# samkatt/fba-pomdp

Measured on AMD Instinct MI355X. Metric: simulated env steps/sec (belief+rollout), higher is better.
Workload: dtype f64

## Files before the change

fba_pomdp_amd/csrc/fba_search.hip:

```cpp
#include <algorithm>
#include <cstdio>
#include <cstdlib>
#include <cstring>

#include "fba_kernels_common.h"

namespace fba {

__device__ __forceinline__ int et_reward_code(double r) { return r == -1.0 ? 0 : (r == 10.0 ? 1 : 2); }
__device__ __forceinline__ double et_reward(int code) { return code == 0 ? -1.0 : (code == 1 ? 10.0 : -100.0); }
#ifdef FBA_PROFILE_SEARCH
__device__ unsigned long long g_search_prof[12];
#define PROF_MARK(r) { const long long now_ = clock64(); prof_[r] += now_ - prev_; prev_ = now_; }
#else
#define PROF_MARK(r)
#endif
template <bool STAGE, int AMAX, bool REG, int TIGER_TABLE, int MODEL, int FTIGER = 0, bool TIGER_POMDP = false, bool FTP = false, bool ETIGER = false>
__global__ void __launch_bounds__(SEARCH_BLOCK) search_kernel(Problem P, DeviceState D)
{
    if (TIGER_POMDP) {
        P.S = 2; P.A = 3; P.O = 2; P.C = 0; P.Cs = 4; P.planner = FBA_PLANNER_POUCT;
        if (P.domain != FBA_DOM_TIGER_CONTINUOUS) P.domain = FBA_DOM_TIGER_EPISODIC;
        P.belief = P.belief == FBA_BELIEF_IMPORTANCE ? FBA_BELIEF_IMPORTANCE : FBA_BELIEF_REJECTION;
        D.cn_off = 1; D.cq_off = 4; D.child_off = 10; D.node_words = 16; D.hash = nullptr;
    }
    P.model = MODEL;
    if (FTIGER > 0) {
        P.S = 1 << FTIGER; P.A = 3; P.O = 2;
        if (P.domain != FBA_DOM_FTIGER_CONTINUOUS) P.domain = FBA_DOM_FTIGER_EPISODIC;
        if (ETIGER) P.domain = FBA_DOM_FTIGER_EPISODIC;
    }
    if (ETIGER) { P.A = 3; P.O = 2; }
    if (TIGER_TABLE) {
        P.model = FBA_MODEL_BA_TABLE; P.planner = FBA_PLANNER_POUCT;
        P.S = 2; P.A = 3; P.O = 2; P.phi_len = 12; P.C = 24; P.Cs = 32;
        if (P.domain != FBA_DOM_TIGER_CONTINUOUS) P.domain = FBA_DOM_TIGER_EPISODIC;
        P.belief = P.belief == FBA_BELIEF_IMPORTANCE ? FBA_BELIEF_IMPORTANCE : FBA_BELIEF_REJECTION;
        D.cn_off = 1; D.cq_off = 4; D.child_off = 10; D.node_words = 16; D.hash = nullptr;
        if (TIGER_TABLE == 2) { P.C = 12; P.Cs = 16; }
    }
    if (ETIGER && (TIGER_TABLE || TIGER_POMDP)) P.domain = FBA_DOM_TIGER_EPISODIC;
    extern __shared__ double lds[];
    __shared__ __attribute__((aligned(8))) float s_prior[TIGER_TABLE == 2 ? 24 : 2];
    const int lane = threadIdx.x;
    const int e    = blockIdx.x * SEARCH_BLOCK + lane;
    if (TIGER_TABLE == 2) {
        if (lane < 24) s_prior[lane] = D.prior_dense[lane];
        __syncthreads();
    }
    if (MODEL == FBA_MODEL_BA_FACTORED && FTIGER == 0) {
        size_t words = search_lds_words(P, D, STAGE, ETIGER);
        words = (words + 3) & ~(size_t)3;
        uint4* dst       = reinterpret_cast<uint4*>(reinterpret_cast<uint32_t*>(lds) + words);
        const uint4* src = reinterpret_cast<const uint4*>(P.fd);
        for (int k = lane; k < (P.fd_bytes + 15) / 16; k += SEARCH_BLOCK) dst[k] = src[k];
        __syncthreads();
        P.fd = reinterpret_cast<const FDesc*>(dst);
    }
    if (e >= P.E || !D.active[e]) return;

    const int depth_cap = P.max_depth > 0 ? P.max_depth : 1;
    float* path_r       = reinterpret_cast<float*>(lds) + lane;
    int32_t* path_na    = reinterpret_cast<int32_t*>(path_r - lane + (size_t)depth_cap * SEARCH_BLOCK) + lane;
    uint16_t* path16    = reinterpret_cast<uint16_t*>(lds) + lane;
    float* stage        = ETIGER ? reinterpret_cast<float*>(lds) + (size_t)((depth_cap + 1) / 2) * SEARCH_BLOCK + lane
                                 : reinterpret_cast<float*>(path_na - lane + (size_t)depth_cap * SEARCH_BLOCK) + lane;
    const bool root_lds = !ETIGER && root_children_in_lds(P, D);
    int16_t* rootch     = reinterpret_cast<int16_t*>(stage - lane + (STAGE ? (size_t)P.Cs * SEARCH_BLOCK : 0)) + lane;
    uint32_t* l1        = reinterpret_cast<uint32_t*>(stage - lane + (STAGE ? (size_t)P.Cs * SEARCH_BLOCK : 0)) + lane;

    Rng g               = slot_rng(P, D, e);
    const int hist_len  = D.t[e];
    const int max_tree_depth = min(P.horizon - hist_len, P.max_depth);
    const int W         = D.node_words;
    int32_t* tree       = D.nodes + (size_t)e * D.max_nodes * W;
    const float* prec   = D.p_rec + pbase(P, e, D.bufsel[e]) * (size_t)P.Cs;

    const bool nested = TIGER_TABLE != 2 && !TIGER_POMDP && !FTP && MODEL != FBA_MODEL_POMDP && P.nested != 0;
    if (P.planner == FBA_PLANNER_RANDOM) {
        g.stream(FBA_PHASE_SEARCH, (uint32_t)P.sims);
        int ns = 0;
        const int src = nested ? nested_sample(P, D, e, g, ns) : belief_sample_uniform(P, D, g);
        D.action[e]   = domain_random_action(P, g, nested ? ns : slot_lazy(D, e) ? lazy_state(P, D, e, src) : rec_state(prec + (size_t)src * P.Cs, P.C));
        return;
    }

    node_init(D, tree, P.A, P.O);
    int n_nodes = 1, tree_depth = 0;
    unsigned long long steps = 0;
    int r_vis = 0, r_cn[AMAX];
    double r_cq[AMAX];
#pragma unroll
    for (int a = 0; a < AMAX; ++a) { r_cn[a] = 0; r_cq[a] = 0.0; }
    if (root_lds)
        for (int k = 0; k < P.A * P.O; ++k) rootch[k * SEARCH_BLOCK] = -1;
    uint32_t l1_exists = 0;
    int4 cy_h2 = make_int4(0, 0, 0, 0), cy_h3 = make_int4(0, 0, 0, 0);
    double cy_q2 = 0, cy_q3 = 0;
    int4* tab      = hash_table(D, e);
    const uint32_t epoch = D.hash ? hash_begin_search(D, e, tab, 0, 1) : 0;

    constexpr bool COMPACT = TIGER_TABLE == 2 && ETIGER;
    const int lazy_c = (slot_lazy(D, e) ? 1 : 0) | (COMPACT && D.compact[e] ? 2 : 0);
    if (COMPACT && (lazy_c & 2)) {
#pragma unroll
        for (int w = 0; w < 10; ++w)
            if (w != 2 && w != 5) stage[w * SEARCH_BLOCK] = 0.f;
    }
    int ts_src = -1, ts_state = 0;
    if (P.planner == FBA_PLANNER_TS) {
        g.stream(FBA_PHASE_SEARCH, (uint32_t)P.sims + 2u);
        ts_src = nested ? nested_sample(P, D, e, g, ts_state) : belief_sample_uniform(P, D, g);
    }
    int sim = -1, mode = 0;
    int s = 0, node = 0, dtg = 0, plen = 0, rdepth = 0;
    const float* cnt = prec;
    double rret = 0, rdisc = 1;
    const int quorum = D.search_quorum;
#ifdef FBA_PROFILE_SEARCH
    long long prof_[12] = {0, 0, 0, 0, 0, 0, 0, 0, 0, 0, 0, 0}, prev_ = clock64();
#endif
    while (true) {
        PROF_MARK(6)
        const bool waiting = mode == 0 && sim < P.sims;
        const int n_wait = __popcll(__ballot(waiting)), n_act = __popcll(__ballot(mode != 0));
        if (n_wait + n_act == 0) break;
        const bool boundary = n_act == 0 || n_wait * 64 >= quorum * (n_wait + n_act);
#ifdef FBA_PROFILE_SEARCH
        const bool lead_ = lane == __ffsll((unsigned long long)__ballot(true)) - 1;
        if (lead_) { prof_[5] += 1; if (boundary) { prof_[9] += 1; prof_[10] += n_wait; } }
#endif
        if (boundary && waiting) {
            double del = rret;
            for (int k = plen - 1; k >= (ETIGER ? 4 : 1); --k) {
                const int na     = ETIGER ? (int)path16[(size_t)k * SEARCH_BLOCK] : path_na[(size_t)k * SEARCH_BLOCK];
                const double ret = (ETIGER ? et_reward(na >> 14) : (double)path_r[(size_t)k * SEARCH_BLOCK]) + P.gamma * del;
                const int act    = ETIGER ? ((na >> 12) & 3) : (na & 31);
                int32_t* rec = tree + (size_t)(ETIGER ? (na & 0xfff) : (na >> 5)) * W;
                double* q    = reinterpret_cast<double*>(rec + D.cq_off) + act;
                int n;
                if (P.A == 3) {
                    int4* hp = reinterpret_cast<int4*>(rec);
                    int4 h   = *hp;
                    n = act == 0 ? ++h.y : (act == 1 ? ++h.z : ++h.w);
                    ++h.x;
                    *hp = h;
                } else {
                    n = ++rec[D.cn_off + act];
                    if (D.cn_off) ++rec[0];
                }
                *q += (ret - *q) / (double)n;
                del = ret;
            }
            if (ETIGER) {
#pragma unroll
                for (int lv = 3; lv >= 2; --lv)
                    if (plen > lv) {
                        const int na     = (int)path16[(size_t)lv * SEARCH_BLOCK];
                        const double ret = et_reward(na >> 14) + P.gamma * del;
                        const int act    = (na >> 12) & 3;
                        int32_t* rec     = tree + (size_t)(na & 0xfff) * W;
                        int4 h           = lv == 3 ? cy_h3 : cy_h2;
                        const double q0  = lv == 3 ? cy_q3 : cy_q2;
                        const int n      = act == 0 ? ++h.y : (act == 1 ? ++h.z : ++h.w);
                        ++h.x;
                        *reinterpret_cast<int4*>(rec) = h;
                        reinterpret_cast<double*>(rec + D.cq_off)[act] = q0 + (ret - q0) / (double)n;
                        del = ret;
                    }
            }
            if (ETIGER && plen > 1) {
                const int na     = (int)path16[1 * SEARCH_BLOCK];
                const double ret = et_reward(na >> 14) + P.gamma * del;
                const int act    = (na >> 12) & 3;
                uint32_t* nd     = l1 + (size_t)(na & 0xfff) * ET_NODE_WORDS * SEARCH_BLOCK;
                uint32_t* cw     = nd + (act >> 1) * SEARCH_BLOCK;
                const uint32_t w = *cw;
                const int n      = (int)((act & 1) ? (w >> 16) : (w & 0xffffu)) + 1;
                *cw              = (act & 1) ? ((w & 0xffffu) | ((uint32_t)n << 16)) : ((w & 0xffff0000u) | (uint32_t)n);
                uint32_t* qw     = nd + (size_t)(3 + 2 * act) * SEARCH_BLOCK;
                double q         = __hiloint2double((int)qw[SEARCH_BLOCK], (int)qw[0]);
                q += (ret - q) / (double)n;
                qw[0]            = (uint32_t)__double2loint(q);
                qw[SEARCH_BLOCK] = (uint32_t)__double2hiint(q);
                del = ret;
            }
            if (plen > 0) {
                const double ret = (ETIGER ? et_reward((int)path16[0] >> 14) : (double)path_r[0]) + P.gamma * del;
                const int act    = ETIGER ? (((int)path16[0] >> 12) & 3) : (path_na[0] & 31);
                int n = 0;
                double q = 0.0;
#pragma unroll
                for (int a2 = 0; a2 < AMAX; ++a2)
                    if (a2 == act) { n = r_cn[a2]; q = r_cq[a2]; }
                ++n;
                q += (ret - q) / (double)n;
#pragma unroll
                for (int a2 = 0; a2 < AMAX; ++a2)
                    if (a2 == act) { r_cn[a2] = n; r_cq[a2] = q; }
                ++r_vis;
            }
            ++sim;
            plen = 0;
        }
        PROF_MARK(4)
        if (boundary && waiting && sim < P.sims) {
            g.stream(FBA_PHASE_SEARCH, (uint32_t)sim);
            int nest_state = ts_state;
            const int src = ts_src >= 0 ? ts_src : (nested ? nested_sample(P, D, e, g, nest_state) : belief_sample_uniform(P, D, g));
            cnt = prec + (size_t)src * P.Cs;
            if (COMPACT && (lazy_c & 2)) {
                const uint4 v = reinterpret_cast<const uint4*>(prec)[src];
                stage[2 * SEARCH_BLOCK]  = __uint_as_float(v.x);
                stage[5 * SEARCH_BLOCK]  = __uint_as_float(v.y);
                stage[10 * SEARCH_BLOCK] = __uint_as_float(v.z);
                stage[11 * SEARCH_BLOCK] = __uint_as_float(v.w & 0x7fffffffu);
                s = (int)(v.w >> 31);
                stage[12 * SEARCH_BLOCK] = __int_as_float(s);
            } else if (STAGE) {
                const float4* rp = reinterpret_cast<const float4*>(cnt);
                const int n4 = (P.C + 4) >> 2;
                constexpr int NB = TIGER_TABLE == 2 ? 4 : 12;
                for (int k0 = 0; k0 < n4; k0 += NB) {
                    float4 v[NB];
#pragma unroll
                    for (int q = 0; q < NB; ++q) v[q] = rp[min(k0 + q, n4 - 1)];
#pragma unroll
                    for (int q = 0; q < NB; ++q) {
                        const int k = k0 + q;
                        if (k < n4) {
                            stage[(4 * k + 0) * SEARCH_BLOCK] = v[q].x;
                            stage[(4 * k + 1) * SEARCH_BLOCK] = v[q].y;
                            stage[(4 * k + 2) * SEARCH_BLOCK] = v[q].z;
                            stage[(4 * k + 3) * SEARCH_BLOCK] = v[q].w;
                        }
                    }
                }
                s = __float_as_int(stage[P.C * SEARCH_BLOCK]);
            } else {
                s = rec_state(cnt, P.C);
            }
            if (lazy_c & 1) s = lazy_state(P, g, src);
            if (nested) s = nest_state;
            node = 0; dtg = max_tree_depth; plen = 0; mode = 1;
        }
        PROF_MARK(0)
        bool finish = false, do_step = mode != 0;
        double delayed = 0;
        int a = 0;
        if (mode == 1) {
            tree_depth = max(tree_depth, max_tree_depth - dtg);
            if (dtg == 0) { finish = true; do_step = false; }
            else if (ETIGER) {
                int cn[AMAX], vis = r_vis;
                double cq[AMAX];
#pragma unroll
                for (int a2 = 0; a2 < AMAX; ++a2) { cn[a2] = r_cn[a2]; cq[a2] = r_cq[a2]; }
                if (node < 0) {
                    const uint32_t* nd = l1 + (size_t)(-1 - node) * ET_NODE_WORDS * SEARCH_BLOCK;
                    const uint32_t w0 = nd[0], w1 = nd[1 * SEARCH_BLOCK];
                    cn[0] = (int)(w0 & 0xffffu); cn[1] = (int)(w0 >> 16); cn[2] = (int)(w1 & 0xffffu);
#pragma unroll
                    for (int a2 = 0; a2 < 3; ++a2)
                        cq[a2] = __hiloint2double((int)nd[(4 + 2 * a2) * SEARCH_BLOCK], (int)nd[(3 + 2 * a2) * SEARCH_BLOCK]);
                    vis = (cn[0] + cn[1]) + cn[2];
                } else if (node > 0) {
                    const int32_t* rec = tree + (size_t)node * W;
                    const int4 h      = *reinterpret_cast<const int4*>(rec);
                    const double2 q01 = *reinterpret_cast<const double2*>(rec + 4);
                    const double q2   = *reinterpret_cast<const double*>(rec + 8);
                    vis = h.x; cn[0] = h.y; cn[1] = h.z; cn[2] = h.w;
                    cq[0] = q01.x; cq[1] = q01.y; cq[2] = q2;
                }
                a = ucb_pick<AMAX>(P, g, D.log1p_tab, vis, cn, cq, true);
                if (plen == 2) { cy_h2 = make_int4(vis, cn[0], cn[1], cn[2]); cy_q2 = a == 0 ? cq[0] : (a == 1 ? cq[1] : cq[2]); }
                if (plen == 3) { cy_h3 = make_int4(vis, cn[0], cn[1], cn[2]); cy_q3 = a == 0 ? cq[0] : (a == 1 ? cq[1] : cq[2]); }
            }
            else if (node == 0) a = ucb_pick<AMAX>(P, g, D.log1p_tab, r_vis, r_cn, r_cq, true);
            else a = ucb_select<AMAX>(P, D, g, tree + (size_t)node * W, true);
        } else if (mode == 2) {
            a = domain_random_action(P, g, s);
        }
        PROF_MARK(1)
        int o;
        double r;
        bool term;
        if (do_step) {
            if (FTIGER > 0 && STAGE && FTP)
                term = ftiger_step_packed<(FTIGER > 0 ? FTIGER : 1)>(P, g, LdsView<SEARCH_BLOCK>{stage}, s, a, o, r, NoInc{});
            else if (FTIGER > 0 && STAGE) term = ftiger_step<(FTIGER > 0 ? FTIGER : 1)>(P, g, LdsView<SEARCH_BLOCK>{stage}, s, a, o, r, NoInc{});
            else if (FTIGER > 0) term = ftiger_step<(FTIGER > 0 ? FTIGER : 1)>(P, g, GlobalSearchView{cnt}, s, a, o, r, NoInc{});
            else if (TIGER_TABLE == 2)
                term = tiger_step_packed(P, g, [&](int w) { return __float_as_uint(stage[w * SEARCH_BLOCK]); }, s_prior, s, a, o, r, NoInc{});
            else if (STAGE) term = sim_step<REG>(P, g, LdsView<SEARCH_BLOCK>{stage}, s, a, o, r, NoInc{});
            else term = sim_step<REG>(P, g, GlobalSearchView{cnt}, s, a, o, r, NoInc{});
            ++steps;
#ifdef FBA_PROFILE_SEARCH
        }
        PROF_MARK(2)
        if (do_step) {
#endif
            if (ETIGER && mode == 1) {
                path16[(size_t)plen * SEARCH_BLOCK] = (uint16_t)((node < 0 ? -1 - node : node) | (a << 12) | (et_reward_code(r) << 14));
                ++plen;
                if (term) finish = true;
                else {
                    int c = 0;
                    if (node == 0) c = ((l1_exists >> o) & 1u) ? -1 - o : 0;
                    else if (node < 0) {
                        const uint32_t w2 = l1[((size_t)(-1 - node) * ET_NODE_WORDS + 2) * SEARCH_BLOCK];
                        c = (int)(o ? (w2 >> 16) : (w2 & 0xffffu));
                    } else {
                        c = tree[(size_t)node * W + D.child_off + 2 * 2 + o];
                        c = c < 0 ? 0 : c;
                    }
                    if (c != 0) { node = c; --dtg; }
                    else {
                        const int nn = min(n_nodes, D.max_nodes - 1);
                        ++n_nodes;
                        if (node == 0) {
                            uint32_t* nd = l1 + (size_t)o * ET_NODE_WORDS * SEARCH_BLOCK;
#pragma unroll
                            for (int k = 0; k < ET_NODE_WORDS; ++k) nd[k * SEARCH_BLOCK] = 0;
                            l1_exists |= 1u << o;
                        } else {
                            node_init(D, tree + (size_t)nn * W, P.A, P.O);
                            if (node < 0) {
                                uint32_t* w2 = l1 + ((size_t)(-1 - node) * ET_NODE_WORDS + 2) * SEARCH_BLOCK;
                                *w2 = o ? ((*w2 & 0xffffu) | ((uint32_t)nn << 16)) : ((*w2 & 0xffff0000u) | (uint32_t)nn);
                            } else tree[(size_t)node * W + D.child_off + 2 * 2 + o] = nn;
                        }
                        mode = 2; rdepth = dtg - 1; rret = 0; rdisc = 1;
                        if (rdepth == 0) finish = true;
                    }
                }
            } else if (mode == 1) {
                path_r[(size_t)plen * SEARCH_BLOCK]  = (float)r;
                path_na[(size_t)plen * SEARCH_BLOCK] = (node << 5) | a  ;
                ++plen;
                if (term) finish = true;
                else {
                    const bool at_root_lds = root_lds && node == 0;
                    const int c = at_root_lds ? rootch[(a * P.O + o) * SEARCH_BLOCK] : child_get(P, D, tree, tab, epoch, node, a, o);
                    if (c >= 0) { node = c; --dtg; }
                    else {
                        const int nn = min(n_nodes, D.max_nodes - 1);
                        ++n_nodes;
                        node_init(D, tree + (size_t)nn * W, P.A, P.O);
                        if (at_root_lds) rootch[(a * P.O + o) * SEARCH_BLOCK] = (int16_t)nn;
                        else child_set(P, D, tree, tab, epoch, node, a, o, nn);
                        mode = 2; rdepth = dtg - 1; rret = 0; rdisc = 1;
                        if (rdepth == 0) finish = true;
                    }
                }
            } else {
                rret += r * rdisc;
                rdisc *= P.gamma;
                --rdepth;
                if (rdepth == 0 || term) { delayed = rret; finish = true; }
            }
        }
        PROF_MARK(3)
        if (finish) { rret = delayed; mode = 0; }
#ifdef FBA_PROFILE_SEARCH
        {
            const int n_step_ = __popcll(__ballot(do_step));
            if (lead_) prof_[8] += n_step_;
        }
#endif
    }
#ifdef FBA_PROFILE_SEARCH
    for (int r = 0; r < 12; ++r)
        if ((r == 5 || r >= 8 ? prof_[r] != 0 : lane == 0) && r != 7 && r != 11) atomicAdd(&g_search_prof[r], (unsigned long long)prof_[r]);
#endif
    g.stream(FBA_PHASE_SEARCH, (uint32_t)P.sims + 1u);
    if (n_nodes > D.max_nodes) atomicCAS(D.fault, 0, -(1 + e));
    const int best = ucb_pick<AMAX>(P, g, D.log1p_tab, 0, r_cn, r_cq, false);
    D.action[e]    = best;
    D.sim_steps[e] += steps;
    fba_trace_rec& rec = D.cur[e];
    rec.n_nodes    = n_nodes;
    rec.tree_depth = tree_depth;
#pragma unroll
    for (int a = 0; a < FBA_MAX_ACTIONS; ++a) {
        rec.root_n[a] = a < AMAX && a < P.A ? r_cn[a < AMAX ? a : 0] : 0;
        rec.root_q[a] = a < AMAX && a < P.A ? r_cq[a < AMAX ? a : 0] : 0.0;
    }
}

template <int K>
__global__ void __launch_bounds__(SEARCH_BLOCK) search_hist_kernel(Problem P, DeviceState D)
{
    constexpr int AMAX = 4;
    P.model = FBA_MODEL_BA_FACTORED; P.domain = FBA_DOM_GRIDWORLD; P.A = 4; P.belief = FBA_BELIEF_IMPORTANCE;
    extern __shared__ double lds[];
    const int lane = threadIdx.x, tl = lane >> 2;
    const int e    = blockIdx.x * HIST_TREES + tl;
    if (e >= P.E || !D.active[e]) return;

    const int depth_cap = P.max_depth > 0 ? P.max_depth : 1;
    double* path_q   = lds + tl;
    int32_t* path_n  = reinterpret_cast<int32_t*>(path_q - tl + (size_t)depth_cap * HIST_TREES) + tl;
    float* path_r    = reinterpret_cast<float*>(path_n - tl + (size_t)depth_cap * HIST_TREES) + tl;
    int32_t* path_na = reinterpret_cast<int32_t*>(path_r - tl + (size_t)depth_cap * HIST_TREES) + tl;
    uint32_t* stage  = reinterpret_cast<uint32_t*>(path_na - tl + (size_t)depth_cap * HIST_TREES) + tl;
    const bool carry = D.cn_off == 0;
    const bool spec = carry && D.max_nodes <= 65538 && P.sims <= 65536;
    int pf_node = -1;
    int4 pf_h = make_int4(0, 0, 0, 0);
    double2 pf_q01 = make_double2(0, 0), pf_q23 = make_double2(0, 0);
    int r_hint[AMAX] = {0, 0, 0, 0};

    QuadRng g;
    g.init(P.seed_lo, P.seed_hi, (uint32_t)D.run[e], (uint32_t)D.episode[e], (uint32_t)D.t[e], lane);
    const int hist_len  = D.t[e];
    const int max_tree_depth = min(P.horizon - hist_len, P.max_depth);
    const int W         = D.node_words;
    int32_t* tree       = D.nodes + (size_t)e * D.max_nodes * W;
    const float* prec   = D.p_rec + rec_base(P, D, e, D.bufsel[e]) * (size_t)P.Cs;
    const uint32_t hist_cnt = D.hist_cnt[e];
    const int hist_n        = hist_total(hist_cnt);
    const uint32_t hist_off = (uint32_t)hist_offset(hist_cnt, 1) << 8 | (uint32_t)hist_offset(hist_cnt, 2) << 16 | (uint32_t)hist_offset(hist_cnt, 3) << 24;

    if (P.planner == FBA_PLANNER_RANDOM) {
        g.stream(FBA_PHASE_SEARCH, (uint32_t)P.sims);
        g.ensure(2);
        (void)g.u01();
        D.action[e] = g.slow_int(0, 4);
        if (P.search_budget > 0) D.search_done[e] = 1;
        return;
    }
    const int budget  = P.search_budget;
    int sim           = budget > 0 ? D.s_sim[e] : 0;
    const bool resume = sim > 0;
    int n_nodes = 1, tree_depth = 0;
    unsigned long long steps = 0;
    int r_vis = 0, r_cn[AMAX];
    double r_cq[AMAX];
#pragma unroll
    for (int a = 0; a < AMAX; ++a) { r_cn[a] = 0; r_cq[a] = 0.0; }
    int4* tab = hash_table(D, e);
    uint32_t epoch;
    if (!resume) {
        node_init(D, tree, P.A, P.O);
        epoch = hash_begin_search(D, e, tab, g.q, HIST_QUAD);
    } else {
        n_nodes    = D.s_nodes[e];
        tree_depth = D.s_depth[e];
        epoch      = D.epoch[e];
        const double* rq = reinterpret_cast<const double*>(tree + D.cq_off);
#pragma unroll
        for (int a = 0; a < AMAX; ++a) { r_cn[a] = tree[D.cn_off + a]; r_cq[a] = rq[a]; r_vis += r_cn[a]; }
    }
    int ts_src = -1;
    if (P.planner == FBA_PLANNER_TS) {
        g.stream(FBA_PHASE_SEARCH, (uint32_t)P.sims + 2u);
        g.ensure(1);
        ts_src = uniform_weight_pick(D.uni_scan, P.N, g.u01() * D.uni_total, D.uni_total);
    }
    int mode = 0, iter = 0;
    int node = 0, dtg = 0, plen = 0, rdepth = 0;
    uint32_t sp = 0, hist_mask = 0;
    double rret = 0, rdisc = 1;
#ifdef FBA_PROFILE_SEARCH
    long long prof_[8] = {0, 0, 0, 0, 0, 0, 0, 0}, prev_ = clock64();
#endif
    while (true) {
        PROF_MARK(6)
        if (mode == 0) {
            if (sim >= P.sims) break;
            if (budget > 0 && iter >= budget) break;
            g.stream(FBA_PHASE_SEARCH, (uint32_t)sim);
            g.ensure(8);
            const int src = ts_src >= 0 ? ts_src : uniform_weight_pick(D.uni_scan, P.N, g.u01() * D.uni_total, D.uni_total);
            const uint4* rp = reinterpret_cast<const uint4*>(prec + (size_t)src * hist_stride(P, hist_n));
            const int n4 = (hist_n + 5) >> 2;
            for (int k0 = g.q; k0 < n4; k0 += 4 * HIST_QUAD) {
                uint4 v[4];
#pragma unroll
                for (int q = 0; q < 4; ++q) v[q] = rp[min(k0 + q * HIST_QUAD, n4 - 1)];
#pragma unroll
                for (int q = 0; q < 4; ++q) {
                    const int k = k0 + q * HIST_QUAD;
                    if (k < n4) {
                        stage[(4 * k + 0) * HIST_TREES] = v[q].x;
                        stage[(4 * k + 1) * HIST_TREES] = v[q].y;
                        stage[(4 * k + 2) * HIST_TREES] = v[q].z;
                        stage[(4 * k + 3) * HIST_TREES] = v[q].w;
                    }
                }
            }
            __builtin_amdgcn_fence(__ATOMIC_ACQ_REL, "wavefront");
            hist_mask = stage[1 * HIST_TREES];
            sp        = (hist_mask >> 16) & 0x3ffu;
            node = 0; dtg = max_tree_depth; plen = 0; mode = 1;
        }
        PROF_MARK(0)
        bool finish = false, do_step = true;
        double delayed = 0;
        int a = 0;
        if (mode == 1 && dtg == 0) { finish = true; do_step = false; }
        if (mode == 1) tree_depth = max(tree_depth, max_tree_depth - dtg);
        int o = 0;
        double r = 0;
        bool term = false;
        if (do_step) {
            g.ensure(7);
            if (mode == 1) {
                int guess = 0;
                if (node == 0) {
                    a = ucb_pick<AMAX>(P, g, D.log1p_tab, r_vis, r_cn, r_cq, true);
                    if (spec) {
                        guess = a == 0 ? r_hint[0] : (a == 1 ? r_hint[1] : (a == 2 ? r_hint[2] : r_hint[3]));
                        if (guess >= min(n_nodes, D.max_nodes)) guess = 0;
                    }
                } else if (carry) {
                    const int32_t* rec = tree + (size_t)node * W;
                    int4 h;
                    double2 q01, q23;
                    if (spec && node == pf_node) { h = pf_h; q01 = pf_q01; q23 = pf_q23; }
                    else {
                        h   = *reinterpret_cast<const int4*>(rec);
                        q01 = *reinterpret_cast<const double2*>(rec + 4);
                        q23 = *reinterpret_cast<const double2*>(rec + 8);
                    }
                    const int m = spec ? 0xffff : -1;
                    const int cn[AMAX]    = {h.x & m, h.y & m, h.z & m, h.w & m};
                    const double cq[AMAX] = {q01.x, q01.y, q23.x, q23.y};
                    a = ucb_pick<AMAX>(P, g, D.log1p_tab, ((cn[0] + cn[1]) + cn[2]) + cn[3], cn, cq, true);
                    const int word = a == 0 ? h.x : (a == 1 ? h.y : (a == 2 ? h.z : h.w));
                    path_n[(size_t)plen * HIST_TREES] = word;
                    path_q[(size_t)plen * HIST_TREES] = a == 0 ? q01.x : (a == 1 ? q01.y : (a == 2 ? q23.x : q23.y));
                    if (spec) {
                        guess = (int)((uint32_t)word >> 16) + 2;
                        if (guess == node || guess >= min(n_nodes, D.max_nodes)) guess = 0;
                    }
                } else a = ucb_select<AMAX>(P, D, g, tree + (size_t)node * W, true);
                if (spec && guess > 0) {
                    const int32_t* crec = tree + (size_t)guess * W;
                    pf_h    = *reinterpret_cast<const int4*>(crec);
                    pf_q01  = *reinterpret_cast<const double2*>(crec + 4);
                    pf_q23  = *reinterpret_cast<const double2*>(crec + 8);
                    pf_node = guess;
                } else pf_node = -1;
            } else {
                a = g.slow_int(0, 4);
            }
#ifdef FBA_PROFILE_SEARCH
        }
        PROF_MARK(1)
        if (do_step) {
#endif
            term = gridworld_hist_step_quad<K, HIST_TREES>(P, g, stage + (size_t)(2 + ((hist_off >> (8 * a)) & 0xffu)) * HIST_TREES,
                                                           hist_count(hist_cnt, a), hist_mask, sp, a, o, r,
                                                           HistRowsGlobal{P.hist_base, P.hist_alt, P.hist_base + HistLayout(P.gw_N, P.gw_G, 4).obase0, HistLayout(P.gw_N, P.gw_G, 4)});
            ++steps;
#ifdef FBA_PROFILE_SEARCH
        }
        PROF_MARK(2)
        if (do_step) {
#endif
            if (mode == 1) {
                path_r[(size_t)plen * HIST_TREES]  = (float)r;
                path_na[(size_t)plen * HIST_TREES] = (node << 5) | a;
                ++plen;
                if (term) finish = true;
                else {
                    const int c = child_get(P, D, tree, tab, epoch, node, a, o);
                    const int nn = min(n_nodes, D.max_nodes - 1);
                    if (spec) {
                        const int to = c >= 0 ? c : nn;
                        if (node == 0) {
#pragma unroll
                            for (int a2 = 0; a2 < AMAX; ++a2)
                                if (a2 == a) r_hint[a2] = to;
                        } else {
                            int32_t* pw = path_n + (size_t)(plen - 1) * HIST_TREES;
                            *pw = (*pw & 0xffff) | (int)((uint32_t)((to - 2) & 0xffff) << 16);
                        }
                    }
                    if (c >= 0) { node = c; --dtg; }
                    else {
                        ++n_nodes;
                        if (spec) {
                            int32_t* nrec = tree + (size_t)nn * W;
                            const int none = (int)((uint32_t)((nn - 2) & 0xffff) << 16);
                            *reinterpret_cast<int4*>(nrec)        = make_int4(none, none, none, none);
                            *reinterpret_cast<double2*>(nrec + 4) = make_double2(0.0, 0.0);
                            *reinterpret_cast<double2*>(nrec + 8) = make_double2(0.0, 0.0);
                        } else node_init(D, tree + (size_t)nn * W, P.A, P.O);
                        child_set(P, D, tree, tab, epoch, node, a, o, nn);
                        mode = 2; rdepth = dtg - 1; rret = 0; rdisc = 1;
                        if (rdepth == 0) finish = true;
                    }
                }
            } else {
                rret += r * rdisc;
                rdisc *= P.gamma;
                --rdepth;
                if (rdepth == 0 || term) { delayed = rret; finish = true; }
            }
        }
        PROF_MARK(3)
        if (finish) {
            double del = delayed;
            for (int k = plen - 1; k >= 0; --k) {
                const int na     = path_na[(size_t)k * HIST_TREES];
                const double ret = (double)path_r[(size_t)k * HIST_TREES] + P.gamma * del;
                const int act    = na & 31;
                if ((na >> 5) == 0) {
                    int n = 0;
                    double q = 0.0;
#pragma unroll
                    for (int a2 = 0; a2 < AMAX; ++a2)
                        if (a2 == act) { n = r_cn[a2]; q = r_cq[a2]; }
                    ++n;
                    q += (ret - q) / (double)n;
#pragma unroll
                    for (int a2 = 0; a2 < AMAX; ++a2)
                        if (a2 == act) { r_cn[a2] = n; r_cq[a2] = q; }
                    ++r_vis;
                } else if (carry) {
                    int32_t* rec    = tree + (size_t)(na >> 5) * W;
                    const int word  = path_n[(size_t)k * HIST_TREES];
                    const int n     = (spec ? (word & 0xffff) : word) + 1;
                    const double q0 = path_q[(size_t)k * HIST_TREES];
                    rec[act] = spec ? ((word & (int)0xffff0000) | n) : n;
                    reinterpret_cast<double*>(rec + D.cq_off)[act] = q0 + (ret - q0) / (double)n;
                } else {
                    int32_t* rec = tree + (size_t)(na >> 5) * W;
                    double* q    = reinterpret_cast<double*>(rec + D.cq_off) + act;
                    const int n  = ++rec[D.cn_off + act];
                    if (D.cn_off) ++rec[0];
                    *q += (ret - *q) / (double)n;
                }
                del = ret;
            }
            ++sim;
            mode = 0;
        }
        PROF_MARK(4)
        ++iter;
#ifdef FBA_PROFILE_SEARCH
        prof_[5] += 1;
#endif
    }
#ifdef FBA_PROFILE_SEARCH
    if (lane == 0)
        for (int r2 = 0; r2 < 8; ++r2) atomicAdd(&g_search_prof[r2], (unsigned long long)prof_[r2]);
#endif
    if (sim < P.sims) {
        double* rq = reinterpret_cast<double*>(tree + D.cq_off);
#pragma unroll
        for (int a = 0; a < AMAX; ++a) { tree[D.cn_off + a] = r_cn[a]; rq[a] = r_cq[a]; }
        if (D.cn_off) tree[0] = r_vis;
        D.s_sim[e]   = sim;
        D.s_nodes[e] = n_nodes;
        D.s_depth[e] = tree_depth;
        if (g.q == 0) D.sim_steps[e] += steps;
        return;
    }
    if (D.s_sim) D.s_sim[e] = 0;
    if (budget > 0) D.search_done[e] = 1;
    g.stream(FBA_PHASE_SEARCH, (uint32_t)P.sims + 1u);
    g.ensure(1);
    if (n_nodes > D.max_nodes) atomicCAS(D.fault, 0, -(1 + e));
    const int best = ucb_pick<AMAX>(P, g, D.log1p_tab, 0, r_cn, r_cq, false);
    D.action[e]    = best;
    if (g.q == 0) D.sim_steps[e] += steps;
    fba_trace_rec& rec = D.cur[e];
    rec.n_nodes    = n_nodes;
    rec.tree_depth = tree_depth;
#pragma unroll
    for (int a = 0; a < FBA_MAX_ACTIONS; ++a) {
        rec.root_n[a] = a < AMAX ? r_cn[a < AMAX ? a : 0] : 0;
        rec.root_q[a] = a < AMAX ? r_cq[a < AMAX ? a : 0] : 0.0;
    }
}

constexpr int H2_PF = 3;

template <int LANE>
__device__ __forceinline__ uint32_t quad_get(uint32_t v)
{
    return (uint32_t)__builtin_amdgcn_mov_dpp((int)v, LANE * 0x55, 0xf, 0xf, true);
}
template <int LANE>
__device__ __forceinline__ double quad_get_f64(uint32_t lo, uint32_t hi)
{
    return __hiloint2double((int)quad_get<LANE>(hi), (int)quad_get<LANE>(lo));
}
__device__ __forceinline__ uint32_t h2_home_line(uint32_t code, uint32_t nlines) { return __umulhi(child_hash((uint64_t)code), nlines); }

#ifndef FBA_HIST2_WAVES
#define FBA_HIST2_WAVES 3
#endif
constexpr int H2_BLOCK = H2_WAVES * 64;
__global__ void __launch_bounds__(1024) search_order_kernel(Problem P, DeviceState D)
{
    __shared__ int32_t s_cnt[258];
    const int tid = threadIdx.x;
    for (int k = tid; k < 258; k += 1024) s_cnt[k] = 0;
    __syncthreads();
    auto key_of = [&](int e) { return D.active[e] ? 1 + min(max(min(P.horizon - D.t[e], P.max_depth), 0), 255) : 0; };
    for (int e = tid; e < P.E; e += 1024) atomicAdd(&s_cnt[key_of(e) + 1], 1);
    __syncthreads();
    if (tid == 0)
        for (int k = 1; k < 258; ++k) s_cnt[k] += s_cnt[k - 1];
    __syncthreads();
    for (int e = tid; e < P.E; e += 1024) D.search_order[atomicAdd(&s_cnt[key_of(e)], 1)] = e;
}

template <int K, bool LROWS>
__global__ void __launch_bounds__(H2_BLOCK) __attribute__((amdgpu_waves_per_eu(FBA_HIST2_WAVES, FBA_HIST2_WAVES))) search_hist2_kernel(Problem P, DeviceState D)
{
    constexpr bool FLAT = false, TAB = false;
#include "fba_search_hist2.inc"
}
template <int K, bool LROWS>
__global__ void __launch_bounds__(H2_BLOCK) __attribute__((amdgpu_waves_per_eu(FBA_HIST2_WAVES, FBA_HIST2_WAVES))) hist2_flat_search(Problem P, DeviceState D)
{
    constexpr bool FLAT = true, TAB = false;
#include "fba_search_hist2.inc"
}
template <bool FLATV>
__global__ void __launch_bounds__(H2_BLOCK) __attribute__((amdgpu_waves_per_eu(FBA_HIST2_WAVES, FBA_HIST2_WAVES))) search_tabhist_kernel(Problem P, DeviceState D)
{
    constexpr bool FLAT = FLATV, TAB = true, LROWS = false;
    constexpr int K = 8;
#include "fba_search_hist2.inc"
}

template <int AMAX>
__global__ void __launch_bounds__(SEARCH_BLOCK) search_ca_hist_kernel(Problem P, DeviceState D)
{
    extern __shared__ uint4 lds4[];
    const int lane = threadIdx.x;
    const int e    = blockIdx.x * SEARCH_BLOCK + lane;
    CaTables T;
    const int tbytes = ca_hist_stage_tables(P, P.hist_row, lds4, lane, SEARCH_BLOCK, T);
    __syncthreads();
    if (e >= P.E || !D.active[e]) return;

    const int depth_cap = P.max_depth > 0 ? P.max_depth : 1;
    float* path_r    = reinterpret_cast<float*>(reinterpret_cast<char*>(lds4) + tbytes) + lane;
    int32_t* path_na = reinterpret_cast<int32_t*>(path_r - lane + (size_t)depth_cap * SEARCH_BLOCK) + lane;
    uint32_t* stage  = reinterpret_cast<uint32_t*>(path_na - lane + (size_t)depth_cap * SEARCH_BLOCK) + lane;

    Rng g               = slot_rng(P, D, e);
    const int hist_len  = D.t[e];
    const int max_tree_depth = min(P.horizon - hist_len, P.max_depth);
    const int W         = D.node_words;
    int32_t* tree       = D.nodes + (size_t)e * D.max_nodes * W;
    const uint32_t hist_cnt = D.hist_cnt[e];
    const int total     = hist_total(hist_cnt), rs = hist_stride(P, total);
    const uint32_t* prec = reinterpret_cast<const uint32_t*>(D.p_rec + rec_base(P, D, e, D.bufsel[e]) * (size_t)P.Cs);

    if (P.planner == FBA_PLANNER_RANDOM) {
        g.stream(FBA_PHASE_SEARCH, (uint32_t)P.sims);
        const int src = belief_sample_uniform(P, D, g);
        D.action[e]   = domain_random_action(P, g, (int)prec[(size_t)src * rs]);
        return;
    }
    node_init(D, tree, P.A, P.O);
    int n_nodes = 1, tree_depth = 0;
    unsigned long long steps = 0;
    int r_vis = 0, r_cn[AMAX];
    double r_cq[AMAX];
#pragma unroll
    for (int a = 0; a < AMAX; ++a) { r_cn[a] = 0; r_cq[a] = 0.0; }
    int4* tab            = hash_table(D, e);
    const uint32_t epoch = D.hash ? hash_begin_search(D, e, tab, 0, 1) : 0;
    const int n4         = (2 + total + 3) >> 2;

    int sim = 0, mode = 0;
    int s = 0, node = 0, dtg = 0, plen = 0, rdepth = 0;
    double rret = 0, rdisc = 1;
    while (true) {
        if (mode == 0) {
            if (sim >= P.sims) break;
            g.stream(FBA_PHASE_SEARCH, (uint32_t)sim);
            const int src   = belief_sample_uniform(P, D, g);
            const uint4* rp = reinterpret_cast<const uint4*>(prec + (size_t)src * rs);
            constexpr int NB = 8;
            for (int k0 = 0; k0 < n4; k0 += NB) {
                uint4 v[NB];
#pragma unroll
                for (int q = 0; q < NB; ++q) v[q] = rp[min(k0 + q, n4 - 1)];
#pragma unroll
                for (int q = 0; q < NB; ++q) {
                    const int k = k0 + q;
                    if (k < n4) {
                        stage[(4 * k + 0) * SEARCH_BLOCK] = v[q].x;
                        stage[(4 * k + 1) * SEARCH_BLOCK] = v[q].y;
                        stage[(4 * k + 2) * SEARCH_BLOCK] = v[q].z;
                        stage[(4 * k + 3) * SEARCH_BLOCK] = v[q].w;
                    }
                }
            }
            s = (int)stage[0];
            node = 0; dtg = max_tree_depth; plen = 0; mode = 1;
        }
        bool finish = false, do_step = true;
        double delayed = 0;
        int a = 0;
        if (mode == 1) {
            tree_depth = max(tree_depth, max_tree_depth - dtg);
            if (dtg == 0) { finish = true; do_step = false; }
            else if (node == 0) a = ucb_pick<AMAX>(P, g, D.log1p_tab, r_vis, r_cn, r_cq, true);
            else a = ucb_select<AMAX>(P, D, g, tree + (size_t)node * W, true);
        } else {
            a = domain_random_action(P, g, s);
        }
        if (do_step) {
            int o;
            double r, unused_prob;
            uint32_t unused_entry;
            const bool term = ca_hist_step<false>(P, g, T, StridedEntries<SEARCH_BLOCK>{stage + (size_t)(2 + hist_offset(hist_cnt, a)) * SEARCH_BLOCK},
                                                  hist_count(hist_cnt, a), s, a, o, r, unused_entry, 0, unused_prob);
            ++steps;
            if (mode == 1) {
                path_r[(size_t)plen * SEARCH_BLOCK]  = (float)r;
                path_na[(size_t)plen * SEARCH_BLOCK] = (node << 5) | a;
                ++plen;
                if (term) finish = true;
                else {
                    const int c = child_get(P, D, tree, tab, epoch, node, a, o);
                    if (c >= 0) { node = c; --dtg; }
                    else {
                        const int nn = min(n_nodes, D.max_nodes - 1);
                        ++n_nodes;
                        node_init(D, tree + (size_t)nn * W, P.A, P.O);
                        child_set(P, D, tree, tab, epoch, node, a, o, nn);
                        mode = 2; rdepth = dtg - 1; rret = 0; rdisc = 1;
                        if (rdepth == 0) finish = true;
                    }
                }
            } else {
                rret += r * rdisc;
                rdisc *= P.gamma;
                --rdepth;
                if (rdepth == 0 || term) { delayed = rret; finish = true; }
            }
        }
        if (finish) {
            double del = delayed;
            for (int k = plen - 1; k >= 1; --k) {
                const int na     = path_na[(size_t)k * SEARCH_BLOCK];
                const double ret = (double)path_r[(size_t)k * SEARCH_BLOCK] + P.gamma * del;
                const int act    = na & 31;
                int32_t* rec = tree + (size_t)(na >> 5) * W;
                double* q    = reinterpret_cast<double*>(rec + D.cq_off) + act;
                const int nv = ++rec[D.cn_off + act];
                if (D.cn_off) ++rec[0];
                *q += (ret - *q) / (double)nv;
                del = ret;
            }
            if (plen > 0) {
                const double ret = (double)path_r[0] + P.gamma * del;
                const int act    = path_na[0] & 31;
                int nv = 0;
                double q = 0.0;
#pragma unroll
                for (int a2 = 0; a2 < AMAX; ++a2)
                    if (a2 == act) { nv = r_cn[a2]; q = r_cq[a2]; }
                ++nv;
                q += (ret - q) / (double)nv;
#pragma unroll
                for (int a2 = 0; a2 < AMAX; ++a2)
                    if (a2 == act) { r_cn[a2] = nv; r_cq[a2] = q; }
                ++r_vis;
            }
            ++sim;
            mode = 0;
        }
    }
    g.stream(FBA_PHASE_SEARCH, (uint32_t)P.sims + 1u);
    if (n_nodes > D.max_nodes) atomicCAS(D.fault, 0, -(1 + e));
    const int best = ucb_pick<AMAX>(P, g, D.log1p_tab, 0, r_cn, r_cq, false);
    D.action[e]    = best;
    D.sim_steps[e] += steps;
    fba_trace_rec& rec = D.cur[e];
    rec.n_nodes    = n_nodes;
    rec.tree_depth = tree_depth;
#pragma unroll
    for (int a = 0; a < FBA_MAX_ACTIONS; ++a) {
        rec.root_n[a] = a < AMAX && a < P.A ? r_cn[a < AMAX ? a : 0] : 0;
        rec.root_q[a] = a < AMAX && a < P.A ? r_cq[a < AMAX ? a : 0] : 0.0;
    }
}

void launch_search(const Problem& P, const DeviceState& D0, hipStream_t st)
{
    const SearchPlan pl = search_plan(P, D0);
    DeviceState D = D0;
    D.search_quorum = (int8_t)pl.quorum;
    static const size_t lds_pad = std::getenv("FBA_SEARCH_LDS_PAD") ? (size_t)std::atoi(std::getenv("FBA_SEARCH_LDS_PAD")) : 0;
    const size_t lds = pl.lds + (kernel_name(pl.kernel) == K_SEARCH ? lds_pad : 0);
    const dim3 grid(pl.grid(P.E)), block(pl.block);
    if (pl.order_first) hipLaunchKernelGGL(search_order_kernel, dim3(1), dim3(1024), 0, st, P, D);
#define FBA_LAUNCH(...)                                                                                                                     \
    {                                                                                                                                       \
        if (pl.raise_lds) (void)hipFuncSetAttribute(reinterpret_cast<const void*>(&__VA_ARGS__), hipFuncAttributeMaxDynamicSharedMemorySize, pl.raise_lds); \
        hipLaunchKernelGGL((__VA_ARGS__), grid, block, lds, st, P, D);                                                                      \
        return;                                                                                                                             \
    }
#define FBA_SEARCH(...) case search_key(__VA_ARGS__): FBA_LAUNCH(search_kernel<__VA_ARGS__>)
#define FBA_HIST_SEARCH(NAME, KERNEL, ...) case kernel_key(NAME, __VA_ARGS__): FBA_LAUNCH(KERNEL<__VA_ARGS__>)
    switch (pl.kernel) {
        FBA_HIST_SEARCH(K_SEARCH_CA_HIST, search_ca_hist_kernel, 4)
        FBA_HIST_SEARCH(K_SEARCH_TABHIST, search_tabhist_kernel, true)
        FBA_HIST_SEARCH(K_SEARCH_TABHIST, search_tabhist_kernel, false)
        FBA_HIST_SEARCH(K_HIST2_FLAT_SEARCH, hist2_flat_search, 8, true)
        FBA_HIST_SEARCH(K_HIST2_FLAT_SEARCH, hist2_flat_search, 8, false)
        FBA_HIST_SEARCH(K_HIST2_FLAT_SEARCH, hist2_flat_search, 12, true)
        FBA_HIST_SEARCH(K_HIST2_FLAT_SEARCH, hist2_flat_search, 12, false)
        FBA_HIST_SEARCH(K_HIST2_FLAT_SEARCH, hist2_flat_search, 16, true)
        FBA_HIST_SEARCH(K_HIST2_FLAT_SEARCH, hist2_flat_search, 16, false)
        FBA_HIST_SEARCH(K_SEARCH_HIST2, search_hist2_kernel, 8, true)
        FBA_HIST_SEARCH(K_SEARCH_HIST2, search_hist2_kernel, 8, false)
        FBA_HIST_SEARCH(K_SEARCH_HIST2, search_hist2_kernel, 12, true)
        FBA_HIST_SEARCH(K_SEARCH_HIST2, search_hist2_kernel, 12, false)
        FBA_HIST_SEARCH(K_SEARCH_HIST2, search_hist2_kernel, 16, true)
        FBA_HIST_SEARCH(K_SEARCH_HIST2, search_hist2_kernel, 16, false)
        FBA_HIST_SEARCH(K_SEARCH_HIST, search_hist_kernel, 8)
        FBA_HIST_SEARCH(K_SEARCH_HIST, search_hist_kernel, 12)
        FBA_HIST_SEARCH(K_SEARCH_HIST, search_hist_kernel, 16)
        FBA_SEARCH(true, 4, false, 2, FBA_MODEL_BA_TABLE, 0, false, false, true)
        FBA_SEARCH(true, 4, false, 2, FBA_MODEL_BA_TABLE, 0, false, false, false)
        FBA_SEARCH(true, 4, false, 1, FBA_MODEL_BA_TABLE, 0, false, false, true)
        FBA_SEARCH(true, 4, false, 1, FBA_MODEL_BA_TABLE, 0, false, false, false)
        FBA_SEARCH(false, 4, false, 0, FBA_MODEL_POMDP, 0, true, false, true)
        FBA_SEARCH(false, 4, false, 0, FBA_MODEL_POMDP, 0, true, false, false)
        FBA_SEARCH(true, 4, false, 0, FBA_MODEL_BA_FACTORED, 2, false, true, true)
        FBA_SEARCH(true, 4, false, 0, FBA_MODEL_BA_FACTORED, 2, false, true, false)
        FBA_SEARCH(true, 4, false, 0, FBA_MODEL_BA_FACTORED, 2)
        FBA_SEARCH(false, 4, false, 0, FBA_MODEL_BA_FACTORED, 2)
        FBA_SEARCH(true, 4, false, 0, FBA_MODEL_BA_FACTORED, 3, false, true, true)
        FBA_SEARCH(true, 4, false, 0, FBA_MODEL_BA_FACTORED, 3, false, true, false)
        FBA_SEARCH(true, 4, false, 0, FBA_MODEL_BA_FACTORED, 3)
        FBA_SEARCH(false, 4, false, 0, FBA_MODEL_BA_FACTORED, 3)
        FBA_SEARCH(true, 4, false, 0, FBA_MODEL_BA_FACTORED, 4, false, true, true)
        FBA_SEARCH(true, 4, false, 0, FBA_MODEL_BA_FACTORED, 4, false, true, false)
        FBA_SEARCH(true, 4, false, 0, FBA_MODEL_BA_FACTORED, 4)
        FBA_SEARCH(false, 4, false, 0, FBA_MODEL_BA_FACTORED, 4)
        FBA_SEARCH(true, 4, true, 0, FBA_MODEL_BA_FACTORED)
        FBA_SEARCH(true, 4, false, 0, FBA_MODEL_BA_FACTORED)
        FBA_SEARCH(true, 4, true, 0, FBA_MODEL_BA_TABLE)
        FBA_SEARCH(true, 4, false, 0, FBA_MODEL_BA_TABLE)
        FBA_SEARCH(false, 4, true, 0, FBA_MODEL_BA_FACTORED)
        FBA_SEARCH(false, 4, false, 0, FBA_MODEL_BA_FACTORED)
        FBA_SEARCH(false, 4, true, 0, FBA_MODEL_BA_TABLE)
        FBA_SEARCH(false, 4, false, 0, FBA_MODEL_BA_TABLE)
        FBA_SEARCH(false, 4, false, 0, FBA_MODEL_POMDP)
        FBA_SEARCH(true, 8, true, 0, FBA_MODEL_BA_FACTORED)
        FBA_SEARCH(true, 8, false, 0, FBA_MODEL_BA_FACTORED)
        FBA_SEARCH(true, 8, true, 0, FBA_MODEL_BA_TABLE)
        FBA_SEARCH(true, 8, false, 0, FBA_MODEL_BA_TABLE)
        FBA_SEARCH(false, 8, true, 0, FBA_MODEL_BA_FACTORED)
        FBA_SEARCH(false, 8, false, 0, FBA_MODEL_BA_FACTORED)
        FBA_SEARCH(false, 8, true, 0, FBA_MODEL_BA_TABLE)
        FBA_SEARCH(false, 8, false, 0, FBA_MODEL_BA_TABLE)
        FBA_SEARCH(false, 8, false, 0, FBA_MODEL_POMDP)
        FBA_SEARCH(true, 16, true, 0, FBA_MODEL_BA_FACTORED)
        FBA_SEARCH(true, 16, false, 0, FBA_MODEL_BA_FACTORED)
        FBA_SEARCH(true, 16, true, 0, FBA_MODEL_BA_TABLE)
        FBA_SEARCH(true, 16, false, 0, FBA_MODEL_BA_TABLE)
        FBA_SEARCH(false, 16, true, 0, FBA_MODEL_BA_FACTORED)
        FBA_SEARCH(false, 16, false, 0, FBA_MODEL_BA_FACTORED)
        FBA_SEARCH(false, 16, true, 0, FBA_MODEL_BA_TABLE)
        FBA_SEARCH(false, 16, false, 0, FBA_MODEL_BA_TABLE)
        FBA_SEARCH(false, 16, false, 0, FBA_MODEL_POMDP)
        FBA_SEARCH(false, 24, false, 0, FBA_MODEL_POMDP)
    }
#undef FBA_HIST_SEARCH
#undef FBA_SEARCH
#undef FBA_LAUNCH
    std::fprintf(stderr, "launch_search: no instantiation behind kernel key %#x\n", pl.kernel);
    std::abort();
}
#ifdef FBA_PROFILE_SEARCH
extern "C" int fba_debug_search_profile(unsigned long long* out, int reset)
{
    if (hipMemcpyFromSymbol(out, HIP_SYMBOL(g_search_prof), sizeof(unsigned long long) * 12) != hipSuccess) return -1;
    if (reset) {
        const unsigned long long z[12] = {0, 0, 0, 0, 0, 0, 0, 0, 0, 0, 0, 0};
        if (hipMemcpyToSymbol(HIP_SYMBOL(g_search_prof), z, sizeof z) != hipSuccess) return -1;
    }
    return 0;
}
#endif

}
```

Baseline: 50.07 billion.

## Peel root step of episodic-tiger search and prefetch next simulation's belief sample

For the episodic tiger path, the next simulation's particle sample and its packed counts are drawn and loaded before the backup loop, so the load latency overlaps the backup work. The root step (UCB pick, environment step, first-level node handling) is peeled out of the main loop and run right after the new simulation starts. This removes the node==0 branches from the generic mode-1 path. It reorders RNG stream usage and restructures control flow, which could change divergence and register pressure.

```diff
diff --git a/fba_pomdp_amd/csrc/fba_search.hip b/fba_pomdp_amd/csrc/fba_search.hip
--- a/fba_pomdp_amd/csrc/fba_search.hip
+++ b/fba_pomdp_amd/csrc/fba_search.hip
@@ -130,6 +130,13 @@
         const bool lead_ = lane == __ffsll((unsigned long long)__ballot(true)) - 1;
         if (lead_) { prof_[5] += 1; if (boundary) { prof_[9] += 1; prof_[10] += n_wait; } }
 #endif
+        int src = 0, nest_state = ts_state;
+        uint4 cv = make_uint4(0, 0, 0, 0);
+        if (ETIGER && boundary && waiting && sim + 1 < P.sims) {
+            g.stream(FBA_PHASE_SEARCH, (uint32_t)(sim + 1));
+            src = ts_src >= 0 ? ts_src : (nested ? nested_sample(P, D, e, g, nest_state) : belief_sample_uniform(P, D, g));
+            if (COMPACT && (lazy_c & 2)) cv = reinterpret_cast<const uint4*>(prec)[src];
+        }
         if (boundary && waiting) {
             double del = rret;
             for (int k = plen - 1; k >= (ETIGER ? 4 : 1); --k) {
@@ -204,13 +211,19 @@
             plen = 0;
         }
         PROF_MARK(4)
-        if (boundary && waiting && sim < P.sims) {
-            g.stream(FBA_PHASE_SEARCH, (uint32_t)sim);
-            int nest_state = ts_state;
-            const int src = ts_src >= 0 ? ts_src : (nested ? nested_sample(P, D, e, g, nest_state) : belief_sample_uniform(P, D, g));
+        const bool start = boundary && waiting && sim < P.sims;
+        int a = 0;
+        if (ETIGER && start && max_tree_depth != 0)
+            a = ucb_pick<AMAX>(P, g, D.log1p_tab, r_vis, r_cn, r_cq, true);
+        PROF_MARK(7)
+        if (start) {
+            if (!ETIGER) {
+                g.stream(FBA_PHASE_SEARCH, (uint32_t)sim);
+                src = ts_src >= 0 ? ts_src : (nested ? nested_sample(P, D, e, g, nest_state) : belief_sample_uniform(P, D, g));
+            }
             cnt = prec + (size_t)src * P.Cs;
             if (COMPACT && (lazy_c & 2)) {
-                const uint4 v = reinterpret_cast<const uint4*>(prec)[src];
+                const uint4 v = cv;
                 stage[2 * SEARCH_BLOCK]  = __uint_as_float(v.x);
                 stage[5 * SEARCH_BLOCK]  = __uint_as_float(v.y);
                 stage[10 * SEARCH_BLOCK] = __uint_as_float(v.z);
@@ -245,17 +258,53 @@
             node = 0; dtg = max_tree_depth; plen = 0; mode = 1;
         }
         PROF_MARK(0)
+        if (ETIGER && start) {
+            if (dtg == 0) { mode = 0; rret = 0; }
+            else {
+                int o;
+                double r;
+                bool term;
+                if (FTIGER > 0 && STAGE && FTP)
+                    term = ftiger_step_packed<(FTIGER > 0 ? FTIGER : 1)>(P, g, LdsView<SEARCH_BLOCK>{stage}, s, a, o, r, NoInc{});
+                else if (FTIGER > 0 && STAGE) term = ftiger_step<(FTIGER > 0 ? FTIGER : 1)>(P, g, LdsView<SEARCH_BLOCK>{stage}, s, a, o, r, NoInc{});
+                else if (FTIGER > 0) term = ftiger_step<(FTIGER > 0 ? FTIGER : 1)>(P, g, GlobalSearchView{cnt}, s, a, o, r, NoInc{});
+                else if (TIGER_TABLE == 2)
+                    term = tiger_step_packed(P, g, [&](int w) {
+                        if (lazy_c & 2) return w == 2 ? cv.x : (w == 5 ? cv.y : (w == 10 ? cv.z : (w == 11 ? cv.w & 0x7fffffffu : 0u)));
+                        return __float_as_uint(stage[w * SEARCH_BLOCK]);
+                    }, s_prior, s, a, o, r, NoInc{});
+                else if (STAGE) term = sim_step<REG>(P, g, LdsView<SEARCH_BLOCK>{stage}, s, a, o, r, NoInc{});
+                else term = sim_step<REG>(P, g, GlobalSearchView{cnt}, s, a, o, r, NoInc{});
+                ++steps;
+#ifdef FBA_PROFILE_SEARCH
+                prof_[11] += 1;
+#endif
+                path16[0] = (uint16_t)((a << 12) | (et_reward_code(r) << 14));
+                plen = 1;
+                if (term) { mode = 0; rret = 0; }
+                else if ((l1_exists >> o) & 1u) { node = -1 - o; --dtg; }
+                else {
+                    ++n_nodes;
+                    uint32_t* nd = l1 + (size_t)o * ET_NODE_WORDS * SEARCH_BLOCK;
+#pragma unroll
+                    for (int k = 0; k < ET_NODE_WORDS; ++k) nd[k * SEARCH_BLOCK] = 0;
+                    l1_exists |= 1u << o;
+                    mode = 2; rdepth = dtg - 1; rret = 0; rdisc = 1;
+                    if (rdepth == 0) mode = 0;
+                }
+            }
+        }
+        PROF_MARK(7)
         bool finish = false, do_step = mode != 0;
         double delayed = 0;
-        int a = 0;
         if (mode == 1) {
             tree_depth = max(tree_depth, max_tree_depth - dtg);
             if (dtg == 0) { finish = true; do_step = false; }
             else if (ETIGER) {
-                int cn[AMAX], vis = r_vis;
+                int cn[AMAX], vis;
                 double cq[AMAX];
 #pragma unroll
-                for (int a2 = 0; a2 < AMAX; ++a2) { cn[a2] = r_cn[a2]; cq[a2] = r_cq[a2]; }
+                for (int a2 = 3; a2 < AMAX; ++a2) { cn[a2] = 0; cq[a2] = 0.0; }
                 if (node < 0) {
                     const uint32_t* nd = l1 + (size_t)(-1 - node) * ET_NODE_WORDS * SEARCH_BLOCK;
                     const uint32_t w0 = nd[0], w1 = nd[1 * SEARCH_BLOCK];
@@ -264,7 +313,7 @@
                     for (int a2 = 0; a2 < 3; ++a2)
                         cq[a2] = __hiloint2double((int)nd[(4 + 2 * a2) * SEARCH_BLOCK], (int)nd[(3 + 2 * a2) * SEARCH_BLOCK]);
                     vis = (cn[0] + cn[1]) + cn[2];
-                } else if (node > 0) {
+                } else {
                     const int32_t* rec = tree + (size_t)node * W;
                     const int4 h      = *reinterpret_cast<const int4*>(rec);
                     const double2 q01 = *reinterpret_cast<const double2*>(rec + 4);
@@ -306,8 +355,7 @@
                 if (term) finish = true;
                 else {
                     int c = 0;
-                    if (node == 0) c = ((l1_exists >> o) & 1u) ? -1 - o : 0;
-                    else if (node < 0) {
+                    if (node < 0) {
                         const uint32_t w2 = l1[((size_t)(-1 - node) * ET_NODE_WORDS + 2) * SEARCH_BLOCK];
                         c = (int)(o ? (w2 >> 16) : (w2 & 0xffffu));
                     } else {
@@ -318,18 +366,11 @@
                     else {
                         const int nn = min(n_nodes, D.max_nodes - 1);
                         ++n_nodes;
-                        if (node == 0) {
-                            uint32_t* nd = l1 + (size_t)o * ET_NODE_WORDS * SEARCH_BLOCK;
-#pragma unroll
-                            for (int k = 0; k < ET_NODE_WORDS; ++k) nd[k * SEARCH_BLOCK] = 0;
-                            l1_exists |= 1u << o;
-                        } else {
-                            node_init(D, tree + (size_t)nn * W, P.A, P.O);
-                            if (node < 0) {
-                                uint32_t* w2 = l1 + ((size_t)(-1 - node) * ET_NODE_WORDS + 2) * SEARCH_BLOCK;
-                                *w2 = o ? ((*w2 & 0xffffu) | ((uint32_t)nn << 16)) : ((*w2 & 0xffff0000u) | (uint32_t)nn);
-                            } else tree[(size_t)node * W + D.child_off + 2 * 2 + o] = nn;
-                        }
+                        node_init(D, tree + (size_t)nn * W, P.A, P.O);
+                        if (node < 0) {
+                            uint32_t* w2 = l1 + ((size_t)(-1 - node) * ET_NODE_WORDS + 2) * SEARCH_BLOCK;
+                            *w2 = o ? ((*w2 & 0xffffu) | ((uint32_t)nn << 16)) : ((*w2 & 0xffff0000u) | (uint32_t)nn);
+                        } else tree[(size_t)node * W + D.child_off + 2 * 2 + o] = nn;
                         mode = 2; rdepth = dtg - 1; rret = 0; rdisc = 1;
                         if (rdepth == 0) finish = true;
                     }
@@ -371,7 +412,7 @@
     }
 #ifdef FBA_PROFILE_SEARCH
     for (int r = 0; r < 12; ++r)
-        if ((r == 5 || r >= 8 ? prof_[r] != 0 : lane == 0) && r != 7 && r != 11) atomicAdd(&g_search_prof[r], (unsigned long long)prof_[r]);
+        if (r == 5 || r >= 8 ? prof_[r] != 0 : lane == 0) atomicAdd(&g_search_prof[r], (unsigned long long)prof_[r]);
 #endif
     g.stream(FBA_PHASE_SEARCH, (uint32_t)P.sims + 1u);
     if (n_nodes > D.max_nodes) atomicCAS(D.fault, 0, -(1 + e));
```

New measurement: 51.57 billion (median of 6 runs). +3.0%, better.
